# thoglu/jammy_flows

Hardware: AMD Instinct MI355X
Metric: log-prob evals/sec (batch 2^20), e4+s2+e4 / gggg+f+gggg (higher is better)
Workload: dtype f32; 1 GPU; pdf("e4+s2+e4","gggg+f+gggg") log-prob, unconditional pdf with autoregressive conditioning, 1048576 rows in total, row-sharded; batch_per_gpu=1048576, total_rows=1048576, parallelism=rows sharded over 1 GPU(s)

## Files before the change

### jammy_flows_amd/csrc/jf_cond_in.h

```cpp
#pragma once
#include "jf_common.h"
#include "jf_math.h"
#include "jf_sphere.h"

namespace jf {

constexpr int JF_COND_IN_MAX = 4;
struct CondIn { int n; jf_cond_segment s[JF_COND_IN_MAX]; };

template <bool FAST> struct CondTrig {
    template <typename T> static __device__ __forceinline__ T sin(T x) { return M<T>::sin(x); }
    template <typename T> static __device__ __forceinline__ T cos(T x) { return M<T>::cos(x); }
};
template <> struct CondTrig<true> {
    static __device__ __forceinline__ float sin(float x) { return __builtin_amdgcn_sinf(x * 0.15915494309189535f); }
    static __device__ __forceinline__ float cos(float x) { return __builtin_amdgcn_cosf(x * 0.15915494309189535f); }
};
template <typename T, bool FAST = false> __device__ __forceinline__ T cond_seg_value(const jf_cond_segment& g, int64_t row, int col) {
    using TR = CondTrig<FAST && std::is_same<T, float>::value>;
    const T* r = static_cast<const T*>(g.src) + row * g.stride;
    if (g.kind == 0) return r[col];
    if (g.kind == 1) return col == 0 ? TR::cos(r[0]) : TR::sin(r[0]);
    if (col == 2) return TR::cos(safe_angle_pi(r[0]));
    return TR::sin(safe_angle_pi(r[0])) * (col == 0 ? TR::cos(r[1]) : TR::sin(r[1]));
}
template <typename T, bool FAST = false> __device__ __forceinline__ T cond_in_value(const CondIn& a, int64_t row, int col) {
    T val = T(0);
#pragma unroll
    for (int i = 0; i < JF_COND_IN_MAX; ++i) {
        if (i < a.n) {
            const int w = a.s[i].kind == 0 ? a.s[i].n_in : a.s[i].kind + 1;
            if (col >= 0 && col < w) val = cond_seg_value<T, FAST>(a.s[i], row, col);
            col -= w;
        }
    }
    return val;
}

template <typename T> struct CondLoc { const T* pa; const T* pb; int kind, col; };
template <typename T> __device__ __forceinline__ CondLoc<T> cond_in_locate(const CondIn& a, int64_t row, int col) {
    CondLoc<T> l;
    const T* r0 = static_cast<const T*>(a.s[0].src) + row * a.s[0].stride;
    l.pa = r0; l.pb = r0; l.kind = 0; l.col = 0;
#pragma unroll
    for (int i = 0; i < JF_COND_IN_MAX; ++i) {
        if (i < a.n) {
            const int kind = a.s[i].kind;
            const int w = kind == 0 ? a.s[i].n_in : kind + 1;
            const bool here = col >= 0 && col < w;
            const T* r = static_cast<const T*>(a.s[i].src) + row * a.s[i].stride;
            const T* pa = r + (kind == 0 ? col : 0);
            const T* pb = r + (kind == 2 ? 1 : (kind == 0 ? col : 0));
            l.pa = here ? pa : l.pa; l.pb = here ? pb : l.pb; l.kind = here ? kind : l.kind; l.col = here ? col : l.col;
            col -= w;
        }
    }
    return l;
}
template <typename T, bool FAST> __device__ __forceinline__ T cond_in_finish(const CondLoc<T>& l, T va, T vb, bool any_embed) {
    if (!any_embed) return va;
    using TR = CondTrig<FAST && std::is_same<T, float>::value>;
    const T th = l.kind == 2 ? safe_angle_pi(va) : va;
    const T s1 = TR::sin(th), c1 = TR::cos(th), s2 = TR::sin(vb), c2 = TR::cos(vb);
    const T e1 = l.col == 0 ? c1 : s1;
    const T e2 = l.col == 2 ? c1 : s1 * (l.col == 0 ? c2 : s2);
    return l.kind == 0 ? va : (l.kind == 1 ? e1 : e2);
}
__device__ __forceinline__ bool cond_in_any_embed(const CondIn& a) {
    bool e = false;
#pragma unroll
    for (int i = 0; i < JF_COND_IN_MAX; ++i) e = e || (i < a.n && a.s[i].kind != 0);
    return e;
}

static inline int cond_in_make(const jf_cond_segment* segs, int32_t n, int32_t K1, CondIn& out) {
    if (!segs || n < 1 || n > JF_COND_IN_MAX) return n > JF_COND_IN_MAX ? JF_ERR_UNSUPPORTED : JF_ERR_BADARG;
    int w = 0;
    out.n = n;
    for (int i = 0; i < n; ++i) {
        if (!segs[i].src || segs[i].kind < 0 || segs[i].kind > 2 || segs[i].n_in < 0 || segs[i].n_in > JF_MAX_WIDTH) return JF_ERR_BADARG;
        out.s[i] = segs[i];
        w += segs[i].kind == 0 ? segs[i].n_in : segs[i].kind + 1;
    }
    return w == K1 ? JF_OK : JF_ERR_BADARG;
}

}
```

### jammy_flows_amd/csrc/jf_cond_split.h

```cpp
#pragma once
#include "jf_cond_in.h"
#include "jf_cond_regs.h"
#include "jf_mfma.h"

namespace jf {

constexpr int CS_TILES = 9;
static_assert(CS_SLOTS == 4 * CS_TILES, "one register per slot, four registers per tile");
constexpr int CS_CT = 3;
constexpr int CS_CPL = CS_TILES / CS_CT;
constexpr int CS_KSTEPS = 4;
constexpr int CS_NP = 3;
constexpr int CS_FRAG = 1024;
constexpr int CS_W_BYTES = CS_CT * CS_KSTEPS * CS_NP * CS_FRAG;
constexpr int CS_B_BYTES = CS_CT * 16 * 4;
constexpr int CS_CHUNK_BYTES = CS_W_BYTES + CS_B_BYTES;
constexpr int CS_NP16 = 2;
constexpr int CS_W16_BYTES = CS_CT * CS_KSTEPS * CS_NP16 * CS_FRAG;
constexpr int CS_B16_BYTES = CS_B_BYTES + 16;
constexpr int CS_CHUNK16_BYTES = CS_W16_BYTES + CS_B16_BYTES;
constexpr float CS_H_SCALE = 16384.0f;
using f16x8 = __attribute__((ext_vector_type(8))) _Float16;
using f16x2 = __attribute__((ext_vector_type(2))) _Float16;
using f32x2 = __attribute__((ext_vector_type(2))) float;
__device__ __forceinline__ int cs_w_exponent(float wmax) {
    if (!(wmax > 0.f && wmax < INFINITY)) return 0;
    const int e = 14 - ilogbf(wmax);
    return e < -60 ? -60 : (e > 60 ? 60 : e);
}
static __global__ void __launch_bounds__(1024) cs_absmax_kernel(const float* __restrict__ W, int64_t ws, int N, int H, float* __restrict__ out) {
    __shared__ float part[16];
    float m = 0.f;
    const int lane = threadIdx.x & 63, wave = threadIdx.x >> 6;
    if (H == 128 && ws % 4 == 0 && (reinterpret_cast<uintptr_t>(W) & 15u) == 0) {
        const int half = lane >> 5, l4 = (lane & 31) * 4;
        for (int n0 = 8 * wave; n0 < N; n0 += 128) {
            f32x4 v[4];
#pragma unroll
            for (int u = 0; u < 4; ++u) {
                const int n = n0 + 2 * u + half;
                v[u] = n < N ? *reinterpret_cast<const f32x4*>(W + (int64_t)n * ws + l4) : f32x4{0.f, 0.f, 0.f, 0.f};
            }
#pragma unroll
            for (int u = 0; u < 4; ++u) m = fmaxf(fmaxf(m, fmaxf(fabsf(v[u][0]), fabsf(v[u][1]))), fmaxf(fabsf(v[u][2]), fabsf(v[u][3])));
        }
    } else {
        for (int n0 = 4 * wave; n0 < N; n0 += 64) {
            for (int k = lane; k < H; k += 64) {
                float v[4];
#pragma unroll
                for (int u = 0; u < 4; ++u) v[u] = n0 + u < N ? W[(int64_t)(n0 + u) * ws + k] : 0.f;
#pragma unroll
                for (int u = 0; u < 4; ++u) m = fmaxf(m, fabsf(v[u]));
            }
        }
    }
#pragma unroll
    for (int o = 32; o > 0; o >>= 1) m = fmaxf(m, __shfl_xor(m, o));
    if ((threadIdx.x & 63) == 0) part[threadIdx.x >> 6] = m;
    __syncthreads();
    if (threadIdx.x < 4) {
        float t = 0.f;
        if (threadIdx.x == 0) {
#pragma unroll
            for (int w = 0; w < 16; ++w) t = fmaxf(t, part[w]);
        }
        out[threadIdx.x] = t;
    }
}
template <int NP> struct CsGeom;
template <> struct CsGeom<3> { static constexpr int W = CS_W_BYTES, B = CS_B_BYTES, CHUNK = CS_CHUNK_BYTES; };
template <> struct CsGeom<2> { static constexpr int W = CS_W16_BYTES, B = CS_B16_BYTES, CHUNK = CS_CHUNK16_BYTES; };
__device__ __forceinline__ void cs_split16(float v0, float v1, unsigned& hi, unsigned& lo) {
    const f16x2 h = __builtin_convertvector(f32x2{v0, v1}, f16x2);
    const f32x2 back = __builtin_convertvector(h, f32x2);
    const f16x2 l = __builtin_convertvector(f32x2{v0 - back[0], v1 - back[1]}, f16x2);
    hi = __builtin_bit_cast(unsigned, h);
    lo = __builtin_bit_cast(unsigned, l);
}
constexpr int CS_ROWS1 = 64;
constexpr int CS_HMAX = 128, CS_K1MAX = 28;

template <typename Op> __device__ __forceinline__ float cs_rreduce(float v, Op op) {
    float a = v, b = v;
    asm("s_nop 1\n\tv_permlane16_swap_b32 %0, %1" : "+v"(a), "+v"(b));
    float c = op(a, b), e = c;
    asm("s_nop 1\n\tv_permlane32_swap_b32 %0, %1" : "+v"(c), "+v"(e));
    return op(c, e);
}
__device__ __forceinline__ float cs_rsum(float v) { return cs_rreduce(v, [](float a, float b) { return a + b; }); }
template <typename F> __device__ __forceinline__ void cs_rsum4(float a, float b, float c, float d, F f, float (&out)[4]) {
    asm("s_nop 1\n\tv_permlane16_swap_b32 %0, %1\n\tv_permlane16_swap_b32 %2, %3" : "+v"(a), "+v"(b), "+v"(c), "+v"(d));
    float ab = a + b, cd = c + d;
    asm("s_nop 1\n\tv_permlane32_swap_b32 %0, %1" : "+v"(ab), "+v"(cd));
    float t = f(ab + cd), t2 = t;
    asm("s_nop 1\n\tv_permlane32_swap_b32 %0, %1" : "+v"(t), "+v"(t2));
    float t1 = t, t3 = t2;
    asm("s_nop 1\n\tv_permlane16_swap_b32 %0, %1\n\tv_permlane16_swap_b32 %2, %3" : "+v"(t), "+v"(t1), "+v"(t2), "+v"(t3));
    out[0] = t; out[1] = t1; out[2] = t2; out[3] = t3;
}
__device__ __forceinline__ float cs_rmax(float v) { return cs_rreduce(v, [](float a, float b) { return fmaxf(a, b); }); }

static inline bool cs_layer_supported(const jf_gf_layer& h, int D) {
    return h.num_kde == CS_K && h.hh_iter >= 0 && h.hh_iter <= CS_HH && h.nonlinear_stretch_type == JF_GF_STRETCH_CLASSIC &&
           h.rotation_mode == JF_GF_ROT_HOUSEHOLDER && !h.center_mean && !h.add_skewness &&
           h.width_mode == JF_GF_WIDTH_SMOOTH_SATURATION && !h.clamp_widths && h.fit_normalization && h.regulate_normalization &&
           h.width_min > 0 && h.width_max > 0 && D >= 3 && D <= 4;
}

__device__ __forceinline__ void cs_dma_chunk(__amdgpu_buffer_rsrc_t rsrc, unsigned char* dst, int g, int lane_off, int wave, int lane, int w_bytes,
                                             int b_bytes) {
#pragma unroll
    for (int u = 0; u < CS_W_BYTES / 4096; ++u)
        if (u < w_bytes / 4096) __builtin_amdgcn_raw_ptr_buffer_load_lds(rsrc, (cs_lptr)(dst + (u * 4 + wave) * 1024), 16, lane_off, g + u * 4096, 0, 0);
    if (wave == 0 && lane < b_bytes / 16) __builtin_amdgcn_raw_ptr_buffer_load_lds(rsrc, (cs_lptr)(dst + w_bytes), 16, lane * 16, g + w_bytes, 0, 0);
}

template <int RG, bool STORE_H, int NP = CS_NP>
__device__ __forceinline__ void cs_hidden(const float* __restrict__ in, int64_t in_stride, const float* __restrict__ W1, int64_t w1s,
                                          const float* __restrict__ b1, int K1, int H, int64_t row0, int64_t last, float* Xs,
                                          bf16x8 (&hB)[RG][CS_KSTEPS][NP], float* __restrict__ h_out, int64_t hs, const CondIn* cin = nullptr) {
    using MF = Mfma16<float>;
    constexpr int CS_ROWS = CS_ROWS1 * RG;
    constexpr int MT = 16, KS = 4, NREG = 4, JH = CS_HMAX / MT;
    const int tid = threadIdx.x, lane = tid & 63, wave = tid >> 6;
    const int li = lane & 15, lq = lane >> 4;
    const int k1p = (K1 + KS - 1) / KS * KS, ldk = k1p + 1;
    float* W1s = Xs + CS_ROWS * ldk;
    float* b1s = W1s + CS_HMAX * ldk;
    {
        const int nx = CS_ROWS * k1p, nw = CS_HMAX * k1p;
        if (cin) {
            const bool any_embed = cond_in_any_embed(*cin);
            for (int base = 0; base < nx; base += 4 * 256) {
                CondLoc<float> loc[4]; float va[4], vb[4]; int o[4]; bool keep[4];
#pragma unroll
                for (int u = 0; u < 4; ++u) {
                    const int idx = base + u * 256 + tid;
                    const int r = idx / k1p, c = idx - r * k1p;
                    const int64_t gr = row0 + r;
                    loc[u] = cond_in_locate<float>(*cin, gr <= last ? gr : last, c < K1 ? c : 0);
                    keep[u] = c < K1;
                    o[u] = idx < nx ? r * ldk + c : -1;
                }
#pragma unroll
                for (int u = 0; u < 4; ++u) { va[u] = *loc[u].pa; vb[u] = *loc[u].pb; }
#pragma unroll
                for (int u = 0; u < 4; ++u) {
                    const float t = cond_in_finish<float, true>(loc[u], va[u], vb[u], any_embed);
                    if (o[u] >= 0) Xs[o[u]] = keep[u] ? t : 0.f;
                }
            }
        } else
        for (int base = 0; base < nx; base += 4 * 256) {
            float v[4]; int o[4];
#pragma unroll
            for (int u = 0; u < 4; ++u) {
                const int idx = base + u * 256 + tid;
                const int r = idx / k1p, c = idx - r * k1p;
                const int64_t gr = row0 + r;
                const float t = in[(gr <= last ? gr : last) * in_stride + (c < K1 ? c : 0)];
                v[u] = c < K1 ? t : 0.f;
                o[u] = idx < nx ? r * ldk + c : -1;
            }
#pragma unroll
            for (int u = 0; u < 4; ++u) if (o[u] >= 0) Xs[o[u]] = v[u];
        }
        for (int base = 0; base < nw; base += 4 * 256) {
            float v[4]; int o[4];
#pragma unroll
            for (int u = 0; u < 4; ++u) {
                const int idx = base + u * 256 + tid;
                const int r = idx / k1p, c = idx - r * k1p;
                const float t = W1[(int64_t)(r < H ? r : H - 1) * w1s + (c < K1 ? c : 0)];
                v[u] = (r < H && c < K1) ? t : 0.f;
                o[u] = idx < nw ? r * ldk + c : -1;
            }
#pragma unroll
            for (int u = 0; u < 4; ++u) if (o[u] >= 0) W1s[o[u]] = v[u];
        }
        if (tid < CS_HMAX) b1s[tid] = tid < H ? b1[tid < H ? tid : 0] : 0.f;
    }
    __syncthreads();
#pragma unroll
    for (int g = 0; g < RG; ++g) {
        typename MF::Acc acc[JH];
#pragma unroll
        for (int j = 0; j < JH; ++j)
#pragma unroll
            for (int r = 0; r < NREG; ++r) acc[j][r] = 0.f;
        for (int s = 0; s < k1p / KS; ++s) {
            const int kk = s * KS + lq;
            const float xb = Xs[((wave * RG + g) * MT + li) * ldk + kk];
#pragma unroll
            for (int j = 0; j < JH; ++j) acc[j] = MF::mma(W1s[(j * MT + li) * ldk + kk], xb, acc[j]);
        }
#pragma unroll
        for (int s = 0; s < CS_KSTEPS; ++s) {
            using u32x4 = __attribute__((ext_vector_type(4))) unsigned;
            u32x4 q0, q1, q2;
#pragma unroll
            for (int i = 0; i < 8; i += 2) {
                const int j = 2 * s + (i >> 2), r = i & 3;
                const float h0 = M<float>::tanh_fast(acc[j][r] + b1s[j * MT + 4 * lq + r]);
                const float h1 = M<float>::tanh_fast(acc[j][r + 1] + b1s[j * MT + 4 * lq + r + 1]);
                if constexpr (STORE_H) { acc[j][r] = h0; acc[j][r + 1] = h1; }
                if constexpr (NP == 2) {
                    unsigned ph, pl;
                    cs_split16(h0 * CS_H_SCALE, h1 * CS_H_SCALE, ph, pl);
                    q0[i >> 1] = ph; q1[i >> 1] = pl;
                    continue;
                }
                const unsigned a0 = __builtin_bit_cast(unsigned, h0), a1 = __builtin_bit_cast(unsigned, h1);
                const float r0 = h0 - __builtin_bit_cast(float, a0 & 0xffff0000u), r1 = h1 - __builtin_bit_cast(float, a1 & 0xffff0000u);
                const unsigned c0 = __builtin_bit_cast(unsigned, r0), c1 = __builtin_bit_cast(unsigned, r1);
                const float s0 = r0 - __builtin_bit_cast(float, c0 & 0xffff0000u), s1 = r1 - __builtin_bit_cast(float, c1 & 0xffff0000u);
                q0[i >> 1] = __builtin_amdgcn_perm(a1, a0, 0x07060302u);
                q1[i >> 1] = __builtin_amdgcn_perm(c1, c0, 0x07060302u);
                q2[i >> 1] = __builtin_amdgcn_perm(__builtin_bit_cast(unsigned, s1), __builtin_bit_cast(unsigned, s0), 0x07060302u);
            }
            hB[g][s][0] = __builtin_bit_cast(bf16x8, q0); hB[g][s][1] = __builtin_bit_cast(bf16x8, q1);
            if constexpr (NP == 3) hB[g][s][2] = __builtin_bit_cast(bf16x8, q2);
        }
        if constexpr (STORE_H) {
            const int64_t r = row0 + (wave * RG + g) * MT + li;
            if (r <= last) {
#pragma unroll
                for (int j = 0; j < JH; ++j) {
                    const int c = j * MT + 4 * lq;
                    if (c < H) *reinterpret_cast<f32x4*>(h_out + r * hs + c) = acc[j];
                }
            }
        }
    }
}

}
```

Measured before the change: 1.661 billion log-prob evals/s.

## Restructure conditioner first layer: per-row staging, bias-init MFMA, fused tanh prescale

Staging of the inputs and first-layer weights into shared memory is rewritten. Each thread in the row waves now loads one full conditioning row through a sequential segment walker and computes the sphere embeddings once per segment. The remaining waves load one weight row each, prescaled by 2/ln2 on the fp16 path. Accumulators start from the bias, the MFMA k-loop is fully unrolled across all row groups, and tanh for the split-fp16 path becomes exp2/rcp with an FMA-based hi/lo split. The aim is to cut the index division, redundant trig and extra adds, at the cost of more accumulator registers (RG×JH live) and reliance on wave-role assumptions.

New measurement: 1.718 billion log-prob evals/s, median of 6. +3.4%, better.

```diff
diff --git a/jammy_flows_amd/csrc/jf_cond_in.h b/jammy_flows_amd/csrc/jf_cond_in.h
--- a/jammy_flows_amd/csrc/jf_cond_in.h
+++ b/jammy_flows_amd/csrc/jf_cond_in.h
@@ -73,6 +73,32 @@
     return e;
 }
 
+struct CondWalk {
+    const float* p; int seg, left, kind;
+    __device__ __forceinline__ CondWalk(const float* in, int64_t in_stride, int K1, int64_t row) : p(in + row * in_stride), seg(0), left(K1), kind(0) {}
+    __device__ __forceinline__ CondWalk() : p(nullptr), seg(-1), left(0), kind(0) {}
+    __device__ __forceinline__ void enter(const CondIn& a, int64_t row) {
+        while (left == 0) {
+            ++seg;
+            const void* src = a.s[0].src; int64_t stride = a.s[0].stride; int n_in = a.s[0].n_in;
+            kind = a.s[0].kind;
+#pragma unroll
+            for (int i = 1; i < JF_COND_IN_MAX; ++i)
+                if (seg == i) { src = a.s[i].src; stride = a.s[i].stride; n_in = a.s[i].n_in; kind = a.s[i].kind; }
+            left = kind == 0 ? n_in : kind + 1;
+            p = static_cast<const float*>(src) + row * stride;
+        }
+    }
+    __device__ __forceinline__ void next() { ++p; --left; }
+};
+__device__ __forceinline__ void cond_in_embed(int kind, float va, float vb, float* out) {
+    using TR = CondTrig<true>;
+    const float th = kind == 2 ? safe_angle_pi(va) : va;
+    const float s1 = TR::sin(th), c1 = TR::cos(th);
+    if (kind == 1) { out[0] = c1; out[1] = s1; return; }
+    out[0] = s1 * TR::cos(vb); out[1] = s1 * TR::sin(vb); out[2] = c1;
+}
+
 static inline int cond_in_make(const jf_cond_segment* segs, int32_t n, int32_t K1, CondIn& out) {
     if (!segs || n < 1 || n > JF_COND_IN_MAX) return n > JF_COND_IN_MAX ? JF_ERR_UNSUPPORTED : JF_ERR_BADARG;
     int w = 0;
diff --git a/jammy_flows_amd/csrc/jf_cond_split.h b/jammy_flows_amd/csrc/jf_cond_split.h
--- a/jammy_flows_amd/csrc/jf_cond_split.h
+++ b/jammy_flows_amd/csrc/jf_cond_split.h
@@ -78,6 +78,14 @@
     hi = __builtin_bit_cast(unsigned, h);
     lo = __builtin_bit_cast(unsigned, l);
 }
+__device__ __forceinline__ void cs_split16_plain(float v0, float v1, unsigned& hi, unsigned& lo) {
+    float m = -1.0f;
+    asm("" : "+s"(m));
+    const f16x2 h = __builtin_convertvector(f32x2{v0, v1}, f16x2);
+    const f16x2 l = __builtin_convertvector(f32x2{__builtin_fmaf((float)h[0], m, v0), __builtin_fmaf((float)h[1], m, v1)}, f16x2);
+    hi = __builtin_bit_cast(unsigned, h);
+    lo = __builtin_bit_cast(unsigned, l);
+}
 constexpr int CS_ROWS1 = 64;
 constexpr int CS_HMAX = 128, CS_K1MAX = 28;
 
@@ -122,79 +130,106 @@
                                           bf16x8 (&hB)[RG][CS_KSTEPS][NP], float* __restrict__ h_out, int64_t hs, const CondIn* cin = nullptr) {
     using MF = Mfma16<float>;
     constexpr int CS_ROWS = CS_ROWS1 * RG;
-    constexpr int MT = 16, KS = 4, NREG = 4, JH = CS_HMAX / MT;
+    constexpr int MT = 16, KS = 4, JH = CS_HMAX / MT;
     const int tid = threadIdx.x, lane = tid & 63, wave = tid >> 6;
     const int li = lane & 15, lq = lane >> 4;
     const int k1p = (K1 + KS - 1) / KS * KS, ldk = k1p + 1;
     float* W1s = Xs + CS_ROWS * ldk;
     float* b1s = W1s + CS_HMAX * ldk;
-    {
-        const int nx = CS_ROWS * k1p, nw = CS_HMAX * k1p;
+    constexpr float PRE = NP == 2 ? 2.8853900817779268f : 1.0f;
+    constexpr int CG = 8;
+    const int wv = __builtin_amdgcn_readfirstlane(wave);
+    if (wv * 64 < CS_ROWS) {
+        const int64_t avail = last - row0;
+        const int64_t row = row0 + (tid <= avail ? tid : avail);
+        float ea[JF_COND_IN_MAX], eb[JF_COND_IN_MAX];
         if (cin) {
-            const bool any_embed = cond_in_any_embed(*cin);
-            for (int base = 0; base < nx; base += 4 * 256) {
-                CondLoc<float> loc[4]; float va[4], vb[4]; int o[4]; bool keep[4];
-#pragma unroll
-                for (int u = 0; u < 4; ++u) {
-                    const int idx = base + u * 256 + tid;
-                    const int r = idx / k1p, c = idx - r * k1p;
-                    const int64_t gr = row0 + r;
-                    loc[u] = cond_in_locate<float>(*cin, gr <= last ? gr : last, c < K1 ? c : 0);
-                    keep[u] = c < K1;
-                    o[u] = idx < nx ? r * ldk + c : -1;
-                }
-#pragma unroll
-                for (int u = 0; u < 4; ++u) { va[u] = *loc[u].pa; vb[u] = *loc[u].pb; }
-#pragma unroll
-                for (int u = 0; u < 4; ++u) {
-                    const float t = cond_in_finish<float, true>(loc[u], va[u], vb[u], any_embed);
-                    if (o[u] >= 0) Xs[o[u]] = keep[u] ? t : 0.f;
-                }
-            }
-        } else
-        for (int base = 0; base < nx; base += 4 * 256) {
-            float v[4]; int o[4];
-#pragma unroll
-            for (int u = 0; u < 4; ++u) {
-                const int idx = base + u * 256 + tid;
-                const int r = idx / k1p, c = idx - r * k1p;
-                const int64_t gr = row0 + r;
-                const float t = in[(gr <= last ? gr : last) * in_stride + (c < K1 ? c : 0)];
-                v[u] = c < K1 ? t : 0.f;
-                o[u] = idx < nx ? r * ldk + c : -1;
-            }
-#pragma unroll
-            for (int u = 0; u < 4; ++u) if (o[u] >= 0) Xs[o[u]] = v[u];
-        }
-        for (int base = 0; base < nw; base += 4 * 256) {
-            float v[4]; int o[4];
-#pragma unroll
-            for (int u = 0; u < 4; ++u) {
-                const int idx = base + u * 256 + tid;
-                const int r = idx / k1p, c = idx - r * k1p;
-                const float t = W1[(int64_t)(r < H ? r : H - 1) * w1s + (c < K1 ? c : 0)];
-                v[u] = (r < H && c < K1) ? t : 0.f;
-                o[u] = idx < nw ? r * ldk + c : -1;
-            }
-#pragma unroll
-            for (int u = 0; u < 4; ++u) if (o[u] >= 0) W1s[o[u]] = v[u];
-        }
-        if (tid < CS_HMAX) b1s[tid] = tid < H ? b1[tid < H ? tid : 0] : 0.f;
+#pragma unroll
+            for (int i = 0; i < JF_COND_IN_MAX; ++i) {
+                if (i < cin->n && cin->s[i].kind != 0) {
+                    const float* r = static_cast<const float*>(cin->s[i].src) + row * cin->s[i].stride;
+                    ea[i] = r[0]; eb[i] = r[cin->s[i].kind - 1];
+                }
+            }
+        }
+        float* xr = Xs + tid * ldk;
+        CondWalk w = cin ? CondWalk() : CondWalk(in, in_stride, K1, row);
+        for (int c0 = 0; c0 < k1p; c0 += CG) {
+            float v[CG]; bool plain[CG];
+#pragma unroll
+            for (int u = 0; u < CG; ++u) {
+                plain[u] = false;
+                if (c0 + u < K1) {
+                    if (cin) w.enter(*cin, row);
+                    plain[u] = w.kind == 0;
+                    if (plain[u]) v[u] = *w.p;
+                    w.next();
+                }
+            }
+#pragma unroll
+            for (int u = 0; u < CG; ++u) {
+                if (plain[u]) xr[c0 + u] = v[u];
+                else if (c0 + u >= K1 && c0 + u < k1p) xr[c0 + u] = 0.f;
+            }
+        }
+        if (cin) {
+            int off = 0;
+#pragma unroll
+            for (int i = 0; i < JF_COND_IN_MAX; ++i) {
+                if (i < cin->n) {
+                    const int kind = cin->s[i].kind;
+                    if (kind != 0) {
+                        asm volatile("" : "+v"(ea[i]), "+v"(eb[i]) : : "memory");
+                        cond_in_embed(kind, ea[i], eb[i], xr + off);
+                    }
+                    off += kind == 0 ? cin->s[i].n_in : kind + 1;
+                }
+            }
+        }
+    } else if (wv * 64 < CS_ROWS + CS_HMAX) {
+        const int hu = tid - CS_ROWS, hc = hu < H ? hu : H - 1;
+        const float sc = hu < H ? PRE : 0.f;
+        const float* wr = W1 + (int64_t)hc * w1s;
+        const float b = b1[hc];
+        float* ws = W1s + hu * ldk;
+        for (int c0 = 0; c0 < k1p; c0 += CG) {
+            float v[CG];
+#pragma unroll
+            for (int u = 0; u < CG; ++u)
+                if (c0 + u < K1) v[u] = wr[c0 + u];
+#pragma unroll
+            for (int u = 0; u < CG; ++u) {
+                if (c0 + u < K1) ws[c0 + u] = v[u] * sc;
+                else if (c0 + u < k1p) ws[c0 + u] = 0.f;
+            }
+        }
+        b1s[hu] = b * sc;
     }
     __syncthreads();
+    typename MF::Acc acc[RG][JH];
+#pragma unroll
+    for (int j = 0; j < JH; ++j) {
+        const f32x4 bias = *reinterpret_cast<const f32x4*>(b1s + j * MT + 4 * lq);
+#pragma unroll
+        for (int g = 0; g < RG; ++g) acc[g][j] = bias;
+    }
+#pragma unroll
+    for (int s = 0; s < CS_K1MAX / KS; ++s) {
+        if (s == 0 || s * KS < k1p) {
+            const int kk = s * KS + lq;
+            float xb[RG], wa[JH];
+#pragma unroll
+            for (int g = 0; g < RG; ++g) xb[g] = Xs[((wave * RG + g) * MT + li) * ldk + kk];
+#pragma unroll
+            for (int j = 0; j < JH; ++j) wa[j] = W1s[(j * MT + li) * ldk + kk];
+#pragma unroll
+            for (int j = 0; j < JH; ++j)
+#pragma unroll
+                for (int g = 0; g < RG; ++g) acc[g][j] = MF::mma(wa[j], xb[g], acc[g][j]);
+        }
+    }
 #pragma unroll
     for (int g = 0; g < RG; ++g) {
-        typename MF::Acc acc[JH];
-#pragma unroll
-        for (int j = 0; j < JH; ++j)
-#pragma unroll
-            for (int r = 0; r < NREG; ++r) acc[j][r] = 0.f;
-        for (int s = 0; s < k1p / KS; ++s) {
-            const int kk = s * KS + lq;
-            const float xb = Xs[((wave * RG + g) * MT + li) * ldk + kk];
-#pragma unroll
-            for (int j = 0; j < JH; ++j) acc[j] = MF::mma(W1s[(j * MT + li) * ldk + kk], xb, acc[j]);
-        }
 #pragma unroll
         for (int s = 0; s < CS_KSTEPS; ++s) {
             using u32x4 = __attribute__((ext_vector_type(4))) unsigned;
@@ -202,15 +237,17 @@
 #pragma unroll
             for (int i = 0; i < 8; i += 2) {
                 const int j = 2 * s + (i >> 2), r = i & 3;
-                const float h0 = M<float>::tanh_fast(acc[j][r] + b1s[j * MT + 4 * lq + r]);
-                const float h1 = M<float>::tanh_fast(acc[j][r + 1] + b1s[j * MT + 4 * lq + r + 1]);
-                if constexpr (STORE_H) { acc[j][r] = h0; acc[j][r + 1] = h1; }
                 if constexpr (NP == 2) {
+                    const float t0 = fmaf(-2.0f * CS_H_SCALE, __builtin_amdgcn_rcpf(__builtin_amdgcn_exp2f(acc[g][j][r]) + 1.0f), CS_H_SCALE);
+                    const float t1 = fmaf(-2.0f * CS_H_SCALE, __builtin_amdgcn_rcpf(__builtin_amdgcn_exp2f(acc[g][j][r + 1]) + 1.0f), CS_H_SCALE);
+                    if constexpr (STORE_H) { acc[g][j][r] = t0 * (1.0f / CS_H_SCALE); acc[g][j][r + 1] = t1 * (1.0f / CS_H_SCALE); }
                     unsigned ph, pl;
-                    cs_split16(h0 * CS_H_SCALE, h1 * CS_H_SCALE, ph, pl);
+                    cs_split16_plain(t0, t1, ph, pl);
                     q0[i >> 1] = ph; q1[i >> 1] = pl;
                     continue;
                 }
+                const float h0 = M<float>::tanh_fast(acc[g][j][r]), h1 = M<float>::tanh_fast(acc[g][j][r + 1]);
+                if constexpr (STORE_H) { acc[g][j][r] = h0; acc[g][j][r + 1] = h1; }
                 const unsigned a0 = __builtin_bit_cast(unsigned, h0), a1 = __builtin_bit_cast(unsigned, h1);
                 const float r0 = h0 - __builtin_bit_cast(float, a0 & 0xffff0000u), r1 = h1 - __builtin_bit_cast(float, a1 & 0xffff0000u);
                 const unsigned c0 = __builtin_bit_cast(unsigned, r0), c1 = __builtin_bit_cast(unsigned, r1);
@@ -228,11 +265,11 @@
 #pragma unroll
                 for (int j = 0; j < JH; ++j) {
                     const int c = j * MT + 4 * lq;
-                    if (c < H) *reinterpret_cast<f32x4*>(h_out + r * hs + c) = acc[j];
-                }
-            }
-        }
-    }
-}
-
-}
+                    if (c < H) *reinterpret_cast<f32x4*>(h_out + r * hs + c) = acc[g][j];
+                }
+            }
+        }
+    }
+}
+
+}
```
